# mcahny/vps

Measured on AMD Instinct MI355X. Metric: frames/sec FuseTrack 1024x2048, higher is better.
Workload: dtype f32-grade: f16x3 split operands (fp16 pair with scaled residual, 22 significand bits) on MFMA, f32 accumulate

## Files before the change

vps_amd/csrc/conv_common.h:

```cpp
#pragma once
#include "common.h"
#include "conv_plan.h"
#include <type_traits>
#include <cstdlib>

typedef float f32x16 __attribute__((ext_vector_type(16)));
typedef float f32x4 __attribute__((ext_vector_type(4)));

namespace {


constexpr int BM = 128;
constexpr int BK = 32;
constexpr int LDS_LD = 36;

template <bool X6, typename F>
void with_prec(const int prec, F&& f) {
    if (prec == VPS_PREC_BF16) f(std::integral_constant<int, VPS_PREC_BF16>{});
    else if (prec == VPS_PREC_BF16X3) f(std::integral_constant<int, VPS_PREC_BF16X3>{});
    else if (X6 && prec == VPS_PREC_BF16X6) f(std::integral_constant<int, X6 ? VPS_PREC_BF16X6 : VPS_PREC_F16X3>{});
    else f(std::integral_constant<int, VPS_PREC_F16X3>{});
}

struct RowInfo {
// ... 202 lines not shown
        for (int g = 0; g < 4; ++g)
#pragma unroll
            for (int e = 0; e < 4; ++e) {
                const int co = cbase + b * 32 + 8 * g + e;
                const bool cok = co < d.cout;
                const int cc = min(co, d.cout - 1);
                const float sc = d.scale ? d.scale[cc] : 1.f;
                const float sh = d.shift ? d.shift[cc] : 0.f;
                float rvs[TM];
#pragma unroll
                for (int a = 0; a < TM; ++a) rvs[a] = d_res ? d_res[rpix[a] * d.res_ld + d.res_coff + cc] : 0.f;
#pragma unroll
                for (int a = 0; a < TM; ++a) {
                    if (!inside[a] || !cok) continue;
                    const float t = acc[a][b][4 * g + e] * sc + sh + rvs[a];
                    d.out[opix[a] * d.out_ld + d.out_coff + co] = vps_act(t, d.act, d.slope);
                }
            }
}

typedef __bf16 bf16x8 __attribute__((ext_vector_type(8)));
typedef __bf16 bf16x4 __attribute__((ext_vector_type(4)));
template <class T> using vec8 = T __attribute__((ext_vector_type(8)));
template <class T> using vec4 = T __attribute__((ext_vector_type(4)));
typedef unsigned int u32x4 __attribute__((ext_vector_type(4)));

__device__ __forceinline__ __amdgpu_buffer_rsrc_t make_rsrc(const void* p, const unsigned bytes) {
    return __builtin_amdgcn_make_buffer_rsrc(const_cast<void*>(p), 0, (int)bytes, 0x00020000);
}
template <class V>
__device__ __forceinline__ V buffer_load16(const __amdgpu_buffer_rsrc_t r, const unsigned voff, const unsigned soff) {
    return __builtin_bit_cast(V, __builtin_amdgcn_raw_buffer_load_b128(r, (int)voff, (int)soff, 0));
}
constexpr int LDS_LDH = 32;
__device__ __forceinline__ int lds_swz(int row) { return (row >> 2) & 3; }

template <int MODE> struct Split;
template <> struct Split<VPS_PREC_BF16> {
    typedef __bf16 elem;
    static constexpr int NSA = 1, NSB = 1, NT = 1, NLB = 1;
    static constexpr int PA[6] = {0, 0, 0, 0, 0, 0};
    static constexpr int PB[6] = {0, 0, 0, 0, 0, 0};
};
template <> struct Split<VPS_PREC_BF16X3> {
    typedef __bf16 elem;
    static constexpr int NSA = 2, NSB = 2, NT = 3, NLB = 2;
    static constexpr int PA[6] = {1, 0, 0, 0, 0, 0};
    static constexpr int PB[6] = {0, 1, 0, 0, 0, 0};
};
template <> struct Split<VPS_PREC_BF16X6> {
    typedef __bf16 elem;
    static constexpr int NSA = 3, NSB = 3, NT = 6, NLB = 3;
    static constexpr int PA[6] = {2, 0, 1, 1, 0, 0};
    static constexpr int PB[6] = {0, 2, 1, 0, 1, 0};
};
template <> struct Split<VPS_PREC_F16X3> {
    typedef _Float16 elem;
    static constexpr int NSA = 2, NSB = 3, NT = 3, NLB = 2;
    static constexpr int PA[6] = {0, 1, 0, 0, 0, 0};
    static constexpr int PB[6] = {1, 2, 0, 0, 0, 0};
};

template <int MODE>
__device__ __forceinline__ vec8<typename Split<MODE>::elem> derive_weight_plane(const vec8<typename Split<MODE>::elem> g0) {
    static_assert(MODE == VPS_PREC_F16X3, "only the fp16 mode has a derived weight plane");
    typedef _Float16 h16x8 __attribute__((ext_vector_type(8)));
// ... 58 lines not shown
```

vps_amd/csrc/conv_h8.hip:

```cpp
#include "conv_common.h"

namespace {

template <int MODE, int KH, int KW>
__global__ __launch_bounds__(512, 2)
void conv_mfma_h8_kernel(const vps_conv_desc d, const int tiles_m, const int tiles_n, const int chunks_per_split) {
    constexpr int TM = 2, TN = 2, WAVES_N = 2, BN = 128;
    constexpr int NTAP = KH * KW;
    constexpr int HW = 32 + KW - 1, HH = 8 + KH - 1;
    constexpr int HROWS = HH * HW;
    constexpr int NLD = (HROWS + 63) / 64;
    typedef Split<MODE> SM;
    typedef typename SM::elem elem_t;
    typedef vec8<elem_t> x8;
    typedef vec4<elem_t> x4;
    constexpr int NSA = SM::NSA, NSB = SM::NSB;
    constexpr int PLANE = NLD * 64 * LDS_LDH;
    constexpr int ABUF = NSA * PLANE;
    constexpr int NLB = NSB;
    constexpr int NFRAG = NLB * 2 * (BN / 32);
    constexpr int BBUF = NFRAG * 512;
    static_assert((NFRAG * 64) % 512 == 0, "whole 16-byte chunks per thread");
    constexpr int NBL = NFRAG * 64 / 512;
    static_assert(2 * (ABUF + BBUF) * 2 <= 160 * 1024, "LDS budget of the CU");

    __shared__ __attribute__((aligned(16))) elem_t As[2 * ABUF];
    __shared__ __attribute__((aligned(16))) elem_t Bs[2 * BBUF];

    const int t = threadIdx.x;
    int swz = xcd_swizzle(blockIdx.x, gridDim.x);
    int tile_n, tile_m, cls, split;
    decode_tile(d, swz, tiles_n, tiles_m, tile_n, tile_m, cls, split);

    const int py = cls / d.os_x, px = cls - py * d.os_x;
    const int H = d.H, W = d.W, cin_pad = d.cin_pad;
    const int tiles_x = (d.Qw + 31) >> 5, tiles_y = (d.Qh + 7) >> 3;
    const int tx = tile_m % tiles_x, tq = tile_m / tiles_x;
    const int ty = tq % tiles_y, n = tq / tiles_y;
    const int iy_org = ty * 8 - d.pad_y[py], ix_org = tx * 32 - d.pad_x[px];
// ... 27 lines not shown
        const int iy = iy_org + hy, ix = ix_org + hx;
        const bool ok = hp < HROWS && (unsigned)iy < (unsigned)H && (unsigned)ix < (unsigned)W;
        hoff[i] = ok ? (unsigned)((n * H + iy) * W + ix) * ld4 + (unsigned)(d.in_coff + k4 * 4) * 4u : 0xFFFFFFF0u;
    }

    auto load_A = [&]() {
        const bool kv = achunk * BK + k4 * 4 < cin_pad;
        const unsigned coff = (unsigned)achunk * (BK * 4u);
        ++achunk;
#pragma unroll
        for (int i = 0; i < NLD; ++i)
            areg[i] = buffer_load16<f32x4>(arsrc, (kv && hoff[i] != 0xFFFFFFF0u) ? hoff[i] + coff : 0xFFFFFFF0u, 0u);
    };
    auto store_A = [&](int i, int buf) {
        x4 sp[NSA];
        split_act<MODE>(areg[i], sp, amax);
        const int row = r0 + 64 * i;
#pragma unroll
        for (int p = 0; p < NSA; ++p)
            *reinterpret_cast<x4*>(&As[buf * ABUF + p * PLANE + row * LDS_LDH + (((k4 >> 1) ^ lds_swz(row)) << 3) + ((k4 & 1) << 2)]) = sp[p];
    };
    auto load_B = [&](int step) {
#pragma unroll
        for (int j = 0; j < NBL; ++j) {
            const int f = __builtin_amdgcn_readfirstlane((t + 512 * j) >> 6), bcol = f % (BN / 32), pm = f / (BN / 32);
            breg[j] = buffer_load16<x8>(wrsrc, (unsigned)lane * 16u,
                                        wbase + (unsigned)(((size_t)(pm >> 1) * wplane + ((size_t)bcol * kst + 2 * step + (pm & 1)) * 512) * sizeof(elem_t)));
        }
    };
    auto store_B = [&](int buf) {
#pragma unroll
        for (int j = 0; j < NBL; ++j) *reinterpret_cast<x8*>(&Bs[buf * BBUF + (t + 512 * j) * 8]) = breg[j];
    };

    int hbase[TM];
#pragma unroll
    for (int a = 0; a < TM; ++a) hbase[a] = (wm * TM + a) * HW + (lane & 31);
    x8 af[2][NSA][TM];
    auto read_A = [&](int m, int buf, int toff) {
#pragma unroll
        for (int a = 0; a < TM; ++a) {
            const int hrow = hbase[a] + toff;
            const int off = buf * ABUF + hrow * LDS_LDH + (((2 * m + (lane >> 5)) ^ lds_swz(hrow)) << 3);
#pragma unroll
            for (int p = 0; p < NSA; ++p) af[m][p][a] = *reinterpret_cast<const x8*>(&As[off + p * PLANE]);
        }
    };
    x8 bcur[2][NSB][TN];
    auto read_B = [&](int m, int buf) {
#pragma unroll
        for (int p = 0; p < NLB; ++p)
#pragma unroll
            for (int b = 0; b < TN; ++b)
                bcur[m][p][b] = *reinterpret_cast<const x8*>(&Bs[buf * BBUF + (((p * 2 + m) * (BN / 32)) + wn * TN + b) * 512 + lane * 8]);
        if constexpr (NLB < NSB) {
#pragma unroll
            for (int b = 0; b < TN; ++b) bcur[m][2][b] = derive_weight_plane<MODE>(bcur[m][0][b]);
        }
    };

    f32x16 acc[TM][TN];
#pragma unroll
    for (int a = 0; a < TM; ++a)
#pragma unroll
        for (int b = 0; b < TN; ++b)
#pragma unroll
            for (int r = 0; r < 16; ++r) acc[a][b][r] = 0.f;

    load_A();
    load_B(0);
#pragma unroll
    for (int i = 0; i < NLD; ++i) store_A(i, 0);
    store_B(0);
    load_A();
    __syncthreads();

    constexpr int NT = SM::NT;
    constexpr int NMF = 2 * NT * TM * TN;
    constexpr int SPT = (NLD + NTAP - 2) / (NTAP - 1);
    constexpr int NW = SPT + 3;

    for (int chunk = 0; chunk < nchunks; ++chunk) {
        const int cur = chunk & 1;
#pragma unroll
        for (int tp = 0; tp < NTAP; ++tp) {
            const int step = chunk * NTAP + tp;
            const int bb = step & 1;
            const int bstep = min(step + 1, nsteps - 1);
            const int toff = (tp / KW) * HW + (tp % KW);
            read_A(0, cur, toff);
            read_B(0, bb);
            __builtin_amdgcn_sched_barrier(0);

            auto work = [&](const int w) {
                if (w == 0) load_B(bstep);
                else if (w == 1) { read_A(1, cur, toff); read_B(1, bb); }
                else if (w < SPT + 2) {
                    const int si = w - 2;
                    if (tp < NTAP - 1) {
                        const int row = tp * SPT + si;
                        if (row < NLD) store_A(row, cur ^ 1);
                    } else if (si == 0) load_A();
                } else store_B(bb ^ 1);
            };

            int mf = 0;
#pragma unroll
            for (int m = 0; m < 2; ++m)
#pragma unroll
                for (int q = 0; q < NT; ++q)
#pragma unroll
                    for (int a = 0; a < TM; ++a)
#pragma unroll
                        for (int b = 0; b < TN; ++b) {
                            acc[a][b] = split_mfma<MODE>(bcur[m][SM::PB[q]][b], af[m][SM::PA[q]][a], acc[a][b]);
                            ++mf;
#pragma unroll
                            for (int w = 0; w < NW; ++w) {
                                const int pos = ((w + 1) * NMF) / (NW + 1);
                                if (mf == (pos < 1 ? 1 : pos)) {
                                    __builtin_amdgcn_sched_barrier(0);
                                    work(w);
                                    __builtin_amdgcn_sched_barrier(0);
                                }
                            }
                        }
            __syncthreads();
        }
    }
    report_range<MODE>(d, amax);
    conv_epilogue<TM, TN, BN, true, 5>(d, acc, tiles_m * 256, tile_m, tile_n, cls, split, py, px, wm, wn, lane, (cls * tiles_m + tile_m) * tiles_n + tile_n);
}

struct S2Tap { int ph, j, i, idx, t, nt; };
constexpr int s2_taps_1d(int K, int a) { return (K - a + 1) / 2; }
constexpr S2Tap s2_tap(int K, int ts) {
    int base = 0;
    for (int ph = 0; ph < 4; ++ph) {
        const int a = ph >> 1, b = ph & 1, J = s2_taps_1d(K, a), I = s2_taps_1d(K, b);
        if (ts < base + J * I) {
            const int t = ts - base, j = t / I, i = t - j * I;
            return S2Tap{ph, j, i, (2 * j + a) * K + 2 * i + b, t, J * I};
        }
        base += J * I;
    }
    return S2Tap{0, 0, 0, 0, 0, 1};
}
template <int N, typename F>
__device__ __forceinline__ void static_for(F&& f) {
    if constexpr (N > 0) {
        static_for<N - 1>(f);
        f(std::integral_constant<int, N - 1>{});
    }
}

template <int MODE, int K, int BN = 128>
__global__ __launch_bounds__(512, 2)
void conv_mfma_h8s2_kernel(const vps_conv_desc d, const int tiles_m, const int tiles_n, const int chunks_per_split) {
    static_assert(BN == 128 || BN == 64, "two column waves of 64 or 32 columns");
    constexpr int TM = 2, TN = BN / 64, WAVES_N = 2;
    constexpr int NTAP = K * K;
    constexpr int J0 = s2_taps_1d(K, 0);
    constexpr int HW = 32 + J0 - 1, HH = 8 + J0 - 1;
    constexpr int HROWS = HH * HW;
    constexpr int NLD = (HROWS + 63) / 64;
    typedef Split<MODE> SM;
    typedef typename SM::elem elem_t;
    typedef vec8<elem_t> x8;
    typedef vec4<elem_t> x4;
    constexpr int NSA = SM::NSA, NSB = SM::NSB;
    constexpr int PLANE = NLD * 64 * LDS_LDH;
    constexpr int ABUF = NSA * PLANE;
    constexpr int NLB = NSB;
    constexpr int NFRAG = NLB * 2 * (BN / 32);
    constexpr int NBL = (NFRAG * 64 + 511) / 512;
    constexpr bool WHOLE = (NFRAG * 64) % 512 == 0;
    constexpr int BBUF = NBL * 512 * 8;
    static_assert(2 * (ABUF + BBUF) * 2 <= 160 * 1024, "LDS budget of the CU");

    __shared__ __attribute__((aligned(16))) elem_t As[2 * ABUF];
    __shared__ __attribute__((aligned(16))) elem_t Bs[2 * BBUF];

    const int t = threadIdx.x;
    const int swz = xcd_swizzle(blockIdx.x, gridDim.x);
    int tile_n, tile_m, cls, split;
    decode_tile(d, swz, tiles_n, tiles_m, tile_n, tile_m, cls, split);

    const int H = d.H, W = d.W, cin_pad = d.cin_pad;
    const int tiles_x = (d.Qw + 31) >> 5, tiles_y = (d.Qh + 7) >> 3;
    const int tx = tile_m % tiles_x, tq = tile_m / tiles_x;
    const int ty = tq % tiles_y, n = tq / tiles_y;
// ... 27 lines not shown
        const unsigned coff = (unsigned)(d.in_coff + cic) * 4u;
        if (++aph == 4) { aph = 0; ++achunk; }
#pragma unroll
        for (int i = 0; i < NLD; ++i) {
            const int hp = r0 + 64 * i;
            const int hy = hp / HW, hx = hp - hy * HW;
            const int iy = iy_org + a + 2 * hy, ix = ix_org + b + 2 * hx;
            const bool ok = kv && hy < rows && hx < cols && (unsigned)iy < (unsigned)H && (unsigned)ix < (unsigned)W;
            areg[i] = buffer_load16<f32x4>(arsrc, ok ? (unsigned)((n * H + iy) * W + ix) * ld4 + coff : 0xFFFFFFF0u, 0u);
        }
    };
    auto store_A = [&](int i, int buf) {
        x4 sp[NSA];
        split_act<MODE>(areg[i], sp, amax);
        const int row = r0 + 64 * i;
#pragma unroll
        for (int p = 0; p < NSA; ++p)
            *reinterpret_cast<x4*>(&As[buf * ABUF + p * PLANE + row * LDS_LDH + (((k4 >> 1) ^ lds_swz(row)) << 3) + ((k4 & 1) << 2)]) = sp[p];
    };
    auto load_B = [&](int wstep) {
#pragma unroll
        for (int j = 0; j < NBL; ++j) {
            const int fr = __builtin_amdgcn_readfirstlane((t + 512 * j) >> 6), f = WHOLE ? fr : min(fr, NFRAG - 1);
            const int bcol = f % (BN / 32), pm = f / (BN / 32);
            breg[j] = buffer_load16<x8>(wrsrc, (unsigned)lane * 16u,
                                        wbase + (unsigned)(((size_t)(pm >> 1) * wplane + ((size_t)bcol * kst + 2 * wstep + (pm & 1)) * 512) * sizeof(elem_t)));
        }
    };
    auto store_B = [&](int buf) {
#pragma unroll
        for (int j = 0; j < NBL; ++j)
            *reinterpret_cast<x8*>(&Bs[buf * BBUF + (t + 512 * j) * 8]) = breg[j];
    };

    int hbase[TM];
#pragma unroll
    for (int a = 0; a < TM; ++a) hbase[a] = (wm * TM + a) * HW + (lane & 31);
    x8 af[2][NSA][TM];
    auto read_A = [&](int m, int buf, int toff) {
#pragma unroll
        for (int a = 0; a < TM; ++a) {
            const int hrow = hbase[a] + toff;
            const int off = buf * ABUF + hrow * LDS_LDH + (((2 * m + (lane >> 5)) ^ lds_swz(hrow)) << 3);
#pragma unroll
            for (int p = 0; p < NSA; ++p) af[m][p][a] = *reinterpret_cast<const x8*>(&As[off + p * PLANE]);
        }
    };
    x8 bcur[2][NSB][TN];
    auto read_B = [&](int m, int buf) {
#pragma unroll
        for (int p = 0; p < NLB; ++p)
#pragma unroll
            for (int b = 0; b < TN; ++b)
                bcur[m][p][b] = *reinterpret_cast<const x8*>(&Bs[buf * BBUF + (((p * 2 + m) * (BN / 32)) + wn * TN + b) * 512 + lane * 8]);
        if constexpr (NLB < NSB) {
#pragma unroll
            for (int b = 0; b < TN; ++b) bcur[m][2][b] = derive_weight_plane<MODE>(bcur[m][0][b]);
        }
    };

    f32x16 acc[TM][TN];
#pragma unroll
    for (int a = 0; a < TM; ++a)
#pragma unroll
        for (int b = 0; b < TN; ++b)
#pragma unroll
            for (int r = 0; r < 16; ++r) acc[a][b][r] = 0.f;

    load_A();
    load_B(s2_tap(K, 0).idx);
#pragma unroll
    for (int i = 0; i < NLD; ++i) store_A(i, 0);
    store_B(0);
    load_A();
    __syncthreads();

    constexpr int NT = SM::NT;
    constexpr int NMF = 2 * NT * TM * TN;

    for (int chunk = 0; chunk < nchunks; ++chunk) {
        static_for<NTAP>([&](auto ts_tag) {
            constexpr int TS = decltype(ts_tag)::value;
            constexpr S2Tap tp = s2_tap(K, TS);
            constexpr S2Tap nx = s2_tap(K, (TS + 1) % NTAP);
            constexpr int cur = tp.ph & 1;
            constexpr bool last_of_phase = tp.t == tp.nt - 1;
            constexpr int SPT = (NLD + tp.nt - 1) / tp.nt;
            constexpr int NW = 3 + SPT + (last_of_phase ? 1 : 0);
            const int step = chunk * NTAP + TS;
            const int bb = step & 1;
            const int wnext = (TS + 1 < NTAP ? chunk : min(chunk + 1, nchunks - 1)) * NTAP + nx.idx;
            constexpr int toff = tp.j * HW + tp.i;
            read_A(0, cur, toff);
            read_B(0, bb);
            __builtin_amdgcn_sched_barrier(0);

            auto work = [&](const int w) {
                if (w == 0) load_B(wnext);
                else if (w == 1) { read_A(1, cur, toff); read_B(1, bb); }
                else if (w < SPT + 2) {
                    const int row = tp.t * SPT + (w - 2);
                    if (row < NLD) store_A(row, cur ^ 1);
                } else if (last_of_phase && w == SPT + 2) load_A();
                else store_B(bb ^ 1);
            };

            int mf = 0;
#pragma unroll
            for (int m = 0; m < 2; ++m)
#pragma unroll
                for (int q = 0; q < NT; ++q)
#pragma unroll
                    for (int a = 0; a < TM; ++a)
#pragma unroll
                        for (int b = 0; b < TN; ++b) {
                            acc[a][b] = split_mfma<MODE>(bcur[m][SM::PB[q]][b], af[m][SM::PA[q]][a], acc[a][b]);
                            ++mf;
#pragma unroll
                            for (int w = 0; w < NW; ++w) {
                                const int pos = ((w + 1) * NMF) / (NW + 1);
                                if (mf == (pos < 1 ? 1 : pos)) {
                                    __builtin_amdgcn_sched_barrier(0);
                                    work(w);
                                    __builtin_amdgcn_sched_barrier(0);
                                }
                            }
                        }
            __syncthreads();
        });
    }
    report_range<MODE>(d, amax);
    conv_epilogue<TM, TN, BN, true, 5>(d, acc, tiles_m * 256, tile_m, tile_n, cls, split, 0, 0, wm, wn, lane, (cls * tiles_m + tile_m) * tiles_n + tile_n);
}

}

__attribute__((visibility("hidden")))
void vpsi_launch_conv_h8(const vps_conv_desc& d, const conv_plan& p, hipStream_t s) {
    with_prec<false>(d.prec, [&](auto mode) {
        constexpr int MODE = decltype(mode)::value;
        if (d.KH == 3) hipLaunchKernelGGL((conv_mfma_h8_kernel<MODE, 3, 3>), dim3(p.grid), dim3(p.block), 0, s, d, p.tiles_m, p.tiles_n, p.chunks_per_split);
        else hipLaunchKernelGGL((conv_mfma_h8_kernel<MODE, 2, 2>), dim3(p.grid), dim3(p.block), 0, s, d, p.tiles_m, p.tiles_n, p.chunks_per_split);
    });
}

__attribute__((visibility("hidden")))
void vpsi_launch_conv_h8s2(const vps_conv_desc& d, const conv_plan& p, hipStream_t s) {
    with_prec<false>(d.prec, [&](auto mode) {
        constexpr int MODE = decltype(mode)::value;
#define VPS_H8S2_LAUNCH(K, BN) \
    hipLaunchKernelGGL((conv_mfma_h8s2_kernel<MODE, K, BN>), dim3(p.grid), dim3(p.block), 0, s, d, p.tiles_m, p.tiles_n, p.chunks_per_split)
        if (d.KH == 3) { if (d.tile_n == 64) VPS_H8S2_LAUNCH(3, 64); else VPS_H8S2_LAUNCH(3, 128); }
        else { if (d.tile_n == 64) VPS_H8S2_LAUNCH(5, 64); else VPS_H8S2_LAUNCH(5, 128); }
#undef VPS_H8S2_LAUNCH
    });
}
```

vps_amd/csrc/conv_h8p.hip:

```cpp
#include "conv_common.h"

namespace {

template <int N, typename F>
__device__ __forceinline__ void static_for_p(F&& f) {
    if constexpr (N > 0) {
        static_for_p<N - 1>(f);
        f(std::integral_constant<int, N - 1>{});
    }
}

template <int MODE, int KH, int KW>
__global__ __launch_bounds__(512, 2)
void conv_mfma_h8p_kernel(const vps_conv_desc d, const int tiles_m, const int tiles_n, const int chunks_per_split) {
    constexpr int TM = 2, TN = 2, WAVES_N = 2, BN = 128;
    constexpr int NTAP = KH * KW;
    static_assert(NTAP % 3 == 0 || NTAP == 4, "ring / register-set index of a tap must be static: 9 taps (9 % 3 == 0) or 4 taps (12-step cycle handled by the caller)");
    constexpr int HW = 32 + KW - 1, HH = 8 + KH - 1;
    constexpr int HROWS = HH * HW;
    constexpr int NLD = (HROWS + 63) / 64;
    typedef Split<MODE> SM;
    typedef typename SM::elem elem_t;
    typedef vec8<elem_t> x8;
    typedef vec4<elem_t> x4;
    constexpr int NSA = SM::NSA, NSB = SM::NSB, NLB = SM::NLB, NT = SM::NT;
    constexpr int PLANE = HROWS * LDS_LDH;
    constexpr int ABUF = NSA * PLANE;
    constexpr int NFRAG = NSB * 2 * (BN / 32);
    constexpr int BBUF = NFRAG * 512;
    static_assert(NFRAG * 64 == NSB * 512, "thread t stages chunk t of every plane");
    static_assert((2 * ABUF + 3 * BBUF) * 2 <= 160 * 1024, "LDS budget of the CU");

    __shared__ __attribute__((aligned(16))) elem_t As[2 * ABUF];
    __shared__ __attribute__((aligned(16))) elem_t Bs[3 * BBUF];

    const int t = threadIdx.x;
    int swz = xcd_swizzle(blockIdx.x, gridDim.x);
    int tile_n, tile_m, cls, split;
    decode_tile(d, swz, tiles_n, tiles_m, tile_n, tile_m, cls, split);

    const int py = cls / d.os_x, px = cls - py * d.os_x;
    const int H = d.H, W = d.W, cin_pad = d.cin_pad;
    const int tiles_x = (d.Qw + 31) >> 5, tiles_y = (d.Qh + 7) >> 3;
    const int tx = tile_m % tiles_x, tq = tile_m / tiles_x;
    const int ty = tq % tiles_y, n = tq / tiles_y;
    const int iy_org = ty * 8 - d.pad_y[py], ix_org = tx * 32 - d.pad_x[px];

    const int k4 = t & 7;
    const int r0 = t >> 3;
    const int chunk0 = split * chunks_per_split;
    const int nchunks = min(chunks_per_split, d.kpad / (BK * NTAP) - chunk0);
    const int nsteps = nchunks * NTAP;

    const int lane = t & 63;
    const int wave = __builtin_amdgcn_readfirstlane(t >> 6);
    const int wm = wave / WAVES_N, wn = wave - wm * WAVES_N;
    const int nbt = d.cout_pad >> 5, kst = d.kpad >> 4;
    const size_t wplane = (size_t)d.nclass * nbt * kst * 512;
    const __amdgpu_buffer_rsrc_t wrsrc = make_rsrc(d.w_split, (unsigned)(wplane * NSB * sizeof(elem_t)));
    const unsigned wbase = (unsigned)((((size_t)(cls * nbt + tile_n * (BN / 32)) * kst + 2 * (size_t)chunk0 * NTAP) * 512) * sizeof(elem_t));
    const __amdgpu_buffer_rsrc_t arsrc = make_rsrc(d.in, (unsigned)((size_t)d.N * H * W * d.in_ld * sizeof(float)));
    const unsigned ld4 = (unsigned)d.in_ld * 4u;

    f32x4 areg[NLD];
    int achunk = chunk0;
    x8 breg[3][NLB];
    float amax = 0.f;

    unsigned hoff[NLD];
#pragma unroll
    for (int i = 0; i < NLD; ++i) {
        const int hp = r0 + 64 * i;
        const int hy = hp / HW, hx = hp - hy * HW;
        const int iy = iy_org + hy, ix = ix_org + hx;
        const bool ok = hp < HROWS && (unsigned)iy < (unsigned)H && (unsigned)ix < (unsigned)W;
        hoff[i] = ok ? (unsigned)((n * H + iy) * W + ix) * ld4 + (unsigned)(d.in_coff + k4 * 4) * 4u : 0xFFFFFFF0u;
    }

    auto load_A = [&]() {
        const bool kv = achunk * BK + k4 * 4 < cin_pad;
        const unsigned coff = (unsigned)achunk * (BK * 4u);
        ++achunk;
#pragma unroll
        for (int i = 0; i < NLD; ++i)
            areg[i] = buffer_load16<f32x4>(arsrc, (kv && hoff[i] != 0xFFFFFFF0u) ? hoff[i] + coff : 0xFFFFFFF0u, 0u);
    };
    auto store_A = [&](const int i, const int buf) {
        x4 sp[NSA];
        split_act<MODE>(areg[i], sp, amax);
        const int row = r0 + 64 * i;
        if (row < HROWS) {
#pragma unroll
            for (int p = 0; p < NSA; ++p)
                *reinterpret_cast<x4*>(&As[buf * ABUF + p * PLANE + row * LDS_LDH + (((k4 >> 1) ^ lds_swz(row)) << 3) + ((k4 & 1) << 2)]) = sp[p];
        }
    };
    auto load_B = [&](const int step, const int set) {
        const int sc = min(step, nsteps - 1);
        const int f = wave, bcol = f % (BN / 32), slab = f / (BN / 32);
#pragma unroll
        for (int p = 0; p < NLB; ++p)
            breg[set][p] = buffer_load16<x8>(wrsrc, (unsigned)lane * 16u,
                                             wbase + (unsigned)(((size_t)p * wplane + ((size_t)bcol * kst + 2 * sc + slab) * 512) * sizeof(elem_t)));
    };
    auto store_B = [&](const int slot, const int set) {
#pragma unroll
        for (int p = 0; p < NLB; ++p) *reinterpret_cast<x8*>(&Bs[slot * BBUF + (t + 512 * p) * 8]) = breg[set][p];
        if constexpr (NLB < NSB) *reinterpret_cast<x8*>(&Bs[slot * BBUF + (t + 512 * NLB) * 8]) = derive_weight_plane<MODE>(breg[set][0]);
    };

    int hbase[TM];
#pragma unroll
    for (int a = 0; a < TM; ++a) hbase[a] = (wm * TM + a) * HW + (lane & 31);
    x8 af[2][NSA][TM];
    x8 bcur[2][NSB][TN];
    constexpr int NRD = NSA * TM + NSB * TN;
    auto read_frag = [&](const int j, const int m, const int abuf, const int toff, const int slot) {
        if (j < NSA * TM) {
            const int p = j / TM, a = j - p * TM;
            const int hrow = hbase[a] + toff;
            af[m][p][a] = *reinterpret_cast<const x8*>(&As[abuf * ABUF + p * PLANE + hrow * LDS_LDH + (((2 * m + (lane >> 5)) ^ lds_swz(hrow)) << 3)]);
        } else {
            const int jj = j - NSA * TM, p = jj / TN, b = jj - p * TN;
            bcur[m][p][b] = *reinterpret_cast<const x8*>(&Bs[slot * BBUF + (((p * 2 + m) * (BN / 32)) + wn * TN + b) * 512 + lane * 8]);
        }
    };

    f32x16 acc[TM][TN];
#pragma unroll
    for (int a = 0; a < TM; ++a)
#pragma unroll
        for (int b = 0; b < TN; ++b)
#pragma unroll
            for (int r = 0; r < 16; ++r) acc[a][b][r] = 0.f;

    load_A();
    load_B(0, 0);
    load_B(1, 1);
#pragma unroll
    for (int i = 0; i < NLD; ++i) store_A(i, 0);
    store_B(0, 0);
    store_B(1, 1);
    load_B(2, 2);
    load_A();
    __syncthreads();
#pragma unroll
    for (int j = 0; j < NRD; ++j) read_frag(j, 0, 0, 0, 0);

    constexpr int NMS = NT * TM * TN;
    constexpr int STG = NTAP / 2;
    constexpr int SPT = (NLD + STG - 1) / STG;
    auto mfma = [&](const int m, const int i) {
        const int q = i / (TM * TN), r = i - q * (TM * TN), a = r / TN, b = r - a * TN;
        acc[a][b] = split_mfma<MODE>(bcur[m][SM::PB[q]][b], af[m][SM::PA[q]][a], acc[a][b]);
    };

    auto tap = [&](const int chunk, auto tp_tag, auto r3_tag) {
        constexpr int tp = decltype(tp_tag)::value;
        constexpr int R3 = decltype(r3_tag)::value;
        const int cur = chunk & 1;
        const int step = chunk * NTAP + tp;
        constexpr int toff = (tp / KW) * HW + (tp % KW);
        constexpr int ntp = (tp + 1) % NTAP;
        constexpr int ntoff = (ntp / KW) * HW + (ntp % KW);
        const int nbuf = tp == NTAP - 1 ? cur ^ 1 : cur;
#pragma unroll
        for (int i = 0; i < NMS; ++i) {
            mfma(0, i);
            __builtin_amdgcn_sched_barrier(0);
            if (i == 0) load_B(step + 3, R3);
#pragma unroll
            for (int j = 0; j < NRD; ++j)
                if ((j * (NMS - 1)) / NRD + 1 == i || (NMS == 1 && i == 0)) read_frag(j, 1, cur, toff, R3);
            __builtin_amdgcn_sched_barrier(0);
        }
#pragma unroll
        for (int i = 0; i < NMS; ++i) {
            mfma(1, i);
            __builtin_amdgcn_sched_barrier(0);
            if (tp < STG) {
#pragma unroll
                for (int si = 0; si < SPT; ++si)
                    if (i == (si * NMS) / (SPT + 1) && tp * SPT + si < NLD) store_A(tp * SPT + si, cur ^ 1);
            }
            if (i == (SPT * NMS) / (SPT + 1)) {
                store_B((R3 + 2) % 3, (R3 + 2) % 3);
                if (tp == STG) load_A();
            }
#pragma unroll
            for (int j = 0; j < NRD; ++j)
                if ((j * (NMS - 1)) / NRD + 1 == i || (NMS == 1 && i == 0)) read_frag(j, 0, nbuf, ntoff, (R3 + 1) % 3);
            __builtin_amdgcn_sched_barrier(0);
        }
        __syncthreads();
    };

    if constexpr (NTAP % 3 == 0) {
        for (int chunk = 0; chunk < nchunks; ++chunk)
            static_for_p<NTAP>([&](auto tpc) {
                constexpr int TP = decltype(tpc)::value;
                tap(chunk, std::integral_constant<int, TP>{}, std::integral_constant<int, TP % 3>{});
            });
    } else {
        int chunk = 0;
        for (; chunk + 2 < nchunks; chunk += 3)
            static_for_p<3 * NTAP>([&](auto sc) {
                constexpr int S = decltype(sc)::value;
                tap(chunk + S / NTAP, std::integral_constant<int, S % NTAP>{}, std::integral_constant<int, S % 3>{});
            });
        if (chunk < nchunks) {
            static_for_p<NTAP>([&](auto sc) {
                constexpr int S = decltype(sc)::value;
                tap(chunk, std::integral_constant<int, S>{}, std::integral_constant<int, S % 3>{});
            });
            ++chunk;
            if (chunk < nchunks)
                static_for_p<NTAP>([&](auto sc) {
                    constexpr int S = decltype(sc)::value;
                    tap(chunk, std::integral_constant<int, S>{}, std::integral_constant<int, (NTAP + S) % 3>{});
                });
        }
    }
    report_range<MODE>(d, amax);
    conv_epilogue<TM, TN, BN, true, 5>(d, acc, tiles_m * 256, tile_m, tile_n, cls, split, py, px, wm, wn, lane, (cls * tiles_m + tile_m) * tiles_n + tile_n);
}

}

__attribute__((visibility("hidden")))
void vpsi_launch_conv_h8p(const vps_conv_desc& d, const conv_plan& p, hipStream_t s) {
    hipLaunchKernelGGL((conv_mfma_h8p_kernel<VPS_PREC_F16X3, 3, 3>), dim3(p.grid), dim3(p.block), 0, s, d, p.tiles_m, p.tiles_n, p.chunks_per_split);
}
```

vps_amd/csrc/conv_mfma.hip:

```cpp
#include "conv_common.h"

namespace {
template <int TM, int TN, int WAVES_M, int WAVES_N, bool DEFORM>
__global__ __launch_bounds__(256, 2)
void conv_mfma_f32_kernel(const vps_conv_desc d, const int M, const int tiles_m, const int tiles_n,
                          const int ksteps_per_split) {
    constexpr int BN = WAVES_N * TN * 32;
    static_assert(WAVES_M * TM * 32 == BM, "block M tile must be 128");
    static_assert(WAVES_M * WAVES_N == 4, "4 wavefronts per block");
    constexpr int NB = BN / 32;

    __shared__ __attribute__((aligned(16))) float As[BM * LDS_LD];
    __shared__ __attribute__((aligned(16))) float Bs[BN * LDS_LD];

    const int t = threadIdx.x;
    int swz = xcd_swizzle(blockIdx.x, gridDim.x);
    int tile_n, tile_m, cls, split;
    decode_tile(d, swz, tiles_n, tiles_m, tile_n, tile_m, cls, split);

    const int py = cls / d.os_x, px = cls - py * d.os_x;
    const int pad_y = d.pad_y[py], pad_x = d.pad_x[px];
    const float* __restrict__ wcls = d.w + (size_t)cls * d.cout_pad * d.kpad;

    const int H = d.H, W = d.W, KH = d.KH, KW = d.KW, cin_pad = d.cin_pad;
// ... 701 lines not shown
}

template <int TM, int TN, int WAVES_M, int WAVES_N>
void launch_conv(const vps_conv_desc& d, const conv_plan& p, hipStream_t s) {
    const dim3 grid(p.grid), block(p.block);
    if (p.kernel == CONV_K_HALO) {
        with_prec<true>(d.prec, [&](auto mode) {
            constexpr int MODE = decltype(mode)::value;
            if (d.KH == 3) hipLaunchKernelGGL((conv_mfma_bf16h_kernel<TM, TN, WAVES_M, WAVES_N, MODE, 3, 3>), grid, block, 0, s, d, p.tiles_m, p.tiles_n, p.chunks_per_split);
            else hipLaunchKernelGGL((conv_mfma_bf16h_kernel<TM, TN, WAVES_M, WAVES_N, MODE, 2, 2>), grid, block, 0, s, d, p.tiles_m, p.tiles_n, p.chunks_per_split);
        });
        return;
    }
#define VPS_CONV_LAUNCH(KERNEL) hipLaunchKernelGGL((KERNEL), grid, block, 0, s, d, p.M, p.tiles_m, p.tiles_n, p.per_split)
    if (p.kernel == CONV_K_F32) {
        if (d.offset) VPS_CONV_LAUNCH((conv_mfma_f32_kernel<TM, TN, WAVES_M, WAVES_N, true>));
        else VPS_CONV_LAUNCH((conv_mfma_f32_kernel<TM, TN, WAVES_M, WAVES_N, false>));
        return;
    }
    const bool tapmajor = d.korder == 0 && d.KH * d.KW > 1;
    with_prec<true>(d.prec, [&](auto mode) {
        constexpr int MODE = decltype(mode)::value;
        if (d.offset) VPS_CONV_LAUNCH((conv_mfma_bf16p_kernel<TM, TN, WAVES_M, WAVES_N, MODE, false, true>));
        else if (tapmajor) VPS_CONV_LAUNCH((conv_mfma_bf16p_kernel<TM, TN, WAVES_M, WAVES_N, MODE, true>));
        else VPS_CONV_LAUNCH((conv_mfma_bf16p_kernel<TM, TN, WAVES_M, WAVES_N, MODE, false>));
    });
#undef VPS_CONV_LAUNCH
}

conv_switches conv_switches_now(const vps_conv_desc& d) {
    const auto on = [](const char* name) { const char* const e = getenv(name); return !(e && atoi(e) == 0); };
    const auto not0 = [](const char* name) { const char* const e = getenv(name); return !(e && e[0] == '0'); };
    static const bool s2_halo = not0("VPS_S2_HALO"), thin = on("VPS_THIN"), debug_occ = getenv("VPS_DEBUG_OCC") != nullptr;
    conv_switches sw = {true, true, true, true, s2_halo, thin, debug_occ};
    if (d.prec != VPS_PREC_F16X3) return sw;
    if (d.tile_n == 32) {
        if (d.cout > 16) sw.n32 = not0("VPS_N32");
        else if (d.nclass == 4) sw.n16t = on("VPS_N16T");
    } else if (d.tile_n <= 128 && d.KH == 1) sw.pw = on("VPS_PW");
    else if (d.tile_n == 128 && d.KH == 3 && d.stride == 1) sw.h8p = on("VPS_H8P");
    return sw;
}

const conv_limits& conv_limits_once(const bool debug) {
    static const conv_limits lim = [debug] {
        conv_limits l = {};
        int dev = 0;
        (void)hipGetDevice(&dev);
        (void)hipDeviceGetAttribute(&l.cus, hipDeviceAttributeMultiprocessorCount, dev);
        vpsi_conv_pw_limits(l, debug);
        vpsi_conv_thin_limits(l, debug);
        if (debug) vpsi_conv_q_debug_occ();
        return l;
    }();
    return lim;
}

}

extern "C" int vps_conv2d(const vps_conv_desc* dp, void* stream) {
    if (!dp) return VPS_EARG(1);
    const vps_conv_desc& d = *dp;
    if (const int e = vpsi_conv_check(d)) return e;
    const conv_switches sw = conv_switches_now(d);
    const conv_plan p = vpsi_conv_plan(d, conv_limits_once(sw.debug_occ), sw);
    hipStream_t s = (hipStream_t)stream;
    switch (p.kernel) {
        case CONV_K_NONE: return p.err;
        case CONV_K_SMALL3X3V: case CONV_K_SMALL_BATCHED: case CONV_K_SMALL: vpsi_launch_conv_small(d, p, s); break;
        case CONV_K_THIN: vpsi_launch_conv_thin(d, p, s); break;
        case CONV_K_DCN256:
            hipLaunchKernelGGL((conv_mfma_bf16p_kernel<2, 4, 2, 2, VPS_PREC_F16X3, false, true>), dim3(p.grid), dim3(p.block), 0, s, d, p.M, p.tiles_m, p.tiles_n, p.per_split);
            break;
        case CONV_K_N16T: case CONV_K_N32: case CONV_K_N16: vpsi_launch_conv_n16(d, p, s); break;
        case CONV_K_H8S2: vpsi_launch_conv_h8s2(d, p, s); break;
        case CONV_K_H8P: vpsi_launch_conv_h8p(d, p, s); break;
        case CONV_K_H8: vpsi_launch_conv_h8(d, p, s); break;
        case CONV_K_PW: vpsi_launch_conv_pw(d, p, s); break;
        case CONV_K_Q: vpsi_launch_conv_q(d, p, s); break;
        default:
            if (d.tile_n == 128) launch_conv<2, 2, 2, 2>(d, p, s);
            else if (d.tile_n == 64) launch_conv<2, 1, 2, 2>(d, p, s);
            else launch_conv<1, 1, 4, 1>(d, p, s);
    }
    int st = vps_launch_status();
    if (st || !p.needs_reduce) return st;
    const size_t total = (size_t)d.nclass * p.M * d.cout;
    if (p.reduce_v4) hipLaunchKernelGGL(conv_splitk_reduce_kernel<4>, dim3(stream_grid((long)(total / 4), 256)), dim3(256), 0, s, d, p.M);
    else hipLaunchKernelGGL(conv_splitk_reduce_kernel<1>, dim3(stream_grid((long)total, 256)), dim3(256), 0, s, d, p.M);
    return vps_launch_status();
}
```

vps_amd/csrc/conv_plan.h:

```cpp
#pragma once
#include <stddef.h>
#include "../../include/vps_hip.h"

#ifndef VPS_EARG
#define VPS_EARG(x) (-1000 - (x))
#endif

enum conv_kernel {
    CONV_K_NONE = 0,
    CONV_K_SMALL3X3V,
    CONV_K_SMALL_BATCHED,
    CONV_K_SMALL,
    CONV_K_THIN,
    CONV_K_DCN256,
    CONV_K_N16T,
    CONV_K_N32,
    CONV_K_N16,
    CONV_K_H8S2,
    CONV_K_H8P,
    CONV_K_H8,
    CONV_K_HALO,
    CONV_K_PW,
    CONV_K_Q,
    CONV_K_F32,
// ... 2 lines not shown

struct conv_plan {
    int kernel;
    int err;
    int M;
    int tiles_m, tiles_n;
    int per_split;
    int chunks_per_split;
    unsigned grid, block;
    size_t smem;
    int nk, nit;
    int G, logG, nslot;
    int runs_per_row, total_runs;
    int thin;
    int ntiles;
    bool needs_reduce;
    bool reduce_v4;
};

struct conv_limits {
    int cus;
    int pw_per_cu[2];
    int thin_per_cu[4];
};

struct conv_switches {
    bool pw;
    bool h8p;
    bool n16t;
    bool n32;
    bool s2_halo;
    bool thin;
    bool debug_occ;
};

struct conv_thin_shape { int c4, ks, s, ph; };
extern const conv_thin_shape conv_thin_shapes[4];

int vpsi_conv_check(const vps_conv_desc& d);
conv_plan vpsi_conv_plan(const vps_conv_desc& d, const conv_limits& lim, const conv_switches& sw);
const char* vpsi_conv_kernel_name(int kernel);

#ifdef __HIPCC__
void vpsi_launch_conv_small(const vps_conv_desc& d, const conv_plan& p, hipStream_t s);
void vpsi_launch_conv_thin(const vps_conv_desc& d, const conv_plan& p, hipStream_t s);
void vpsi_launch_conv_n16(const vps_conv_desc& d, const conv_plan& p, hipStream_t s);
void vpsi_launch_conv_h8(const vps_conv_desc& d, const conv_plan& p, hipStream_t s);
void vpsi_launch_conv_h8p(const vps_conv_desc& d, const conv_plan& p, hipStream_t s);
void vpsi_launch_conv_h8s2(const vps_conv_desc& d, const conv_plan& p, hipStream_t s);
void vpsi_launch_conv_pw(const vps_conv_desc& d, const conv_plan& p, hipStream_t s);
void vpsi_launch_conv_q(const vps_conv_desc& d, const conv_plan& p, hipStream_t s);
void vpsi_conv_pw_limits(conv_limits& lim, bool debug);
void vpsi_conv_thin_limits(conv_limits& lim, bool debug);
void vpsi_conv_q_debug_occ();
#endif
```

Measured before the change: 56.42.

## Stream conv weight tiles straight from global memory into LDS in h8 kernels

```diff
diff --git a/vps_amd/csrc/conv_common.h b/vps_amd/csrc/conv_common.h
--- a/vps_amd/csrc/conv_common.h
+++ b/vps_amd/csrc/conv_common.h
@@ -258,6 +258,21 @@
 __device__ __forceinline__ V buffer_load16(const __amdgpu_buffer_rsrc_t r, const unsigned voff, const unsigned soff) {
     return __builtin_bit_cast(V, __builtin_amdgcn_raw_buffer_load_b128(r, (int)voff, (int)soff, 0));
 }
+__device__ __forceinline__ void glds16(const void* const gbase, const unsigned voff, const unsigned lds_dst) {
+    unsigned keep;
+    asm volatile("s_mov_b32 %0, m0\n\ts_mov_b32 m0, %3\n\ts_nop 0\n\tglobal_load_lds_dwordx4 %1, %2\n\ts_mov_b32 m0, %0"
+                 : "=&s"(keep) : "v"(voff), "s"(gbase), "s"(lds_dst) : "memory");
+}
+template <class T>
+__device__ __forceinline__ unsigned lds_addr(const T* const p) {
+    return (unsigned)__builtin_amdgcn_readfirstlane((int)(size_t)(const __attribute__((address_space(3))) T*)p);
+}
+template <int N>
+__device__ __forceinline__ void wait_vm() {
+    static_assert(N >= 0 && N < 64, "6-bit counter");
+    __builtin_amdgcn_s_waitcnt(0x0F70 | (N & 15) | ((N >> 4) << 14));
+}
+
 constexpr int LDS_LDH = 32;
 __device__ __forceinline__ int lds_swz(int row) { return (row >> 2) & 3; }
 
diff --git a/vps_amd/csrc/conv_h8.hip b/vps_amd/csrc/conv_h8.hip
--- a/vps_amd/csrc/conv_h8.hip
+++ b/vps_amd/csrc/conv_h8.hip
@@ -2,9 +2,8 @@
 
 namespace {
 
-template <int MODE, int KH, int KW>
-__global__ __launch_bounds__(512, 2)
-void conv_mfma_h8_kernel(const vps_conv_desc d, const int tiles_m, const int tiles_n, const int chunks_per_split) {
+template <int MODE, int KH, int KW, bool WDMA>
+__device__ __forceinline__ void conv_h8_body(const vps_conv_desc& d, const int tiles_m, const int tiles_n, const int chunks_per_split) {
     constexpr int TM = 2, TN = 2, WAVES_N = 2, BN = 128;
     constexpr int NTAP = KH * KW;
     constexpr int HW = 32 + KW - 1, HH = 8 + KH - 1;
@@ -98,6 +97,15 @@
 #pragma unroll
         for (int j = 0; j < NBL; ++j) *reinterpret_cast<x8*>(&Bs[buf * BBUF + (t + 512 * j) * 8]) = breg[j];
     };
+    const char* const wsrc = reinterpret_cast<const char*>(d.w_split) + wbase;
+    auto dma_B = [&](int step, int buf) {
+#pragma unroll
+        for (int j = 0; j < NBL; ++j) {
+            const int f = wave + 8 * j, bcol = f % (BN / 32), pm = f / (BN / 32);
+            glds16(wsrc + ((size_t)(pm >> 1) * wplane + ((size_t)bcol * kst + 2 * step + (pm & 1)) * 512) * sizeof(elem_t), (unsigned)lane * 16u,
+                   lds_addr(&Bs[buf * BBUF + f * 512]));
+        }
+    };
 
     int hbase[TM];
 #pragma unroll
@@ -134,11 +142,13 @@
             for (int r = 0; r < 16; ++r) acc[a][b][r] = 0.f;
 
     load_A();
-    load_B(0);
+    if constexpr (WDMA) dma_B(0, 0);
+    else load_B(0);
 #pragma unroll
     for (int i = 0; i < NLD; ++i) store_A(i, 0);
-    store_B(0);
+    if constexpr (!WDMA) store_B(0);
     load_A();
+    if constexpr (WDMA) wait_vm<NLD>();
     __syncthreads();
 
     constexpr int NT = SM::NT;
@@ -159,7 +169,10 @@
             __builtin_amdgcn_sched_barrier(0);
 
             auto work = [&](const int w) {
-                if (w == 0) load_B(bstep);
+                if (w == 0) {
+                    if constexpr (WDMA) dma_B(bstep, bb ^ 1);
+                    else load_B(bstep);
+                }
                 else if (w == 1) { read_A(1, cur, toff); read_B(1, bb); }
                 else if (w < SPT + 2) {
                     const int si = w - 2;
@@ -167,7 +180,7 @@
                         const int row = tp * SPT + si;
                         if (row < NLD) store_A(row, cur ^ 1);
                     } else if (si == 0) load_A();
-                } else store_B(bb ^ 1);
+                } else if constexpr (!WDMA) store_B(bb ^ 1);
             };
 
             int mf = 0;
@@ -191,11 +204,26 @@
                                 }
                             }
                         }
+            if constexpr (WDMA) {
+                if (tp == NTAP - 1) wait_vm<NLD>();
+                else wait_vm<0>();
+            }
             __syncthreads();
         }
     }
     report_range<MODE>(d, amax);
     conv_epilogue<TM, TN, BN, true, 5>(d, acc, tiles_m * 256, tile_m, tile_n, cls, split, py, px, wm, wn, lane, (cls * tiles_m + tile_m) * tiles_n + tile_n);
+}
+
+template <int MODE, int KH, int KW>
+__global__ __launch_bounds__(512, 2)
+void conv_mfma_h8_kernel(const vps_conv_desc d, const int tiles_m, const int tiles_n, const int chunks_per_split) {
+    conv_h8_body<MODE, KH, KW, true>(d, tiles_m, tiles_n, chunks_per_split);
+}
+template <int MODE, int KH, int KW>
+__global__ __launch_bounds__(512, 2)
+void conv_mfma_h8_wreg_kernel(const vps_conv_desc d, const int tiles_m, const int tiles_n, const int chunks_per_split) {
+    conv_h8_body<MODE, KH, KW, false>(d, tiles_m, tiles_n, chunks_per_split);
 }
 
 struct S2Tap { int ph, j, i, idx, t, nt; };
@@ -220,9 +248,8 @@
     }
 }
 
-template <int MODE, int K, int BN = 128>
-__global__ __launch_bounds__(512, 2)
-void conv_mfma_h8s2_kernel(const vps_conv_desc d, const int tiles_m, const int tiles_n, const int chunks_per_split) {
+template <int MODE, int K, int BN, bool WDMA>
+__device__ __forceinline__ void conv_h8s2_body(const vps_conv_desc& d, const int tiles_m, const int tiles_n, const int chunks_per_split) {
     static_assert(BN == 128 || BN == 64, "two column waves of 64 or 32 columns");
     constexpr int TM = 2, TN = BN / 64, WAVES_N = 2;
     constexpr int NTAP = K * K;
@@ -316,6 +343,16 @@
         for (int j = 0; j < NBL; ++j)
             *reinterpret_cast<x8*>(&Bs[buf * BBUF + (t + 512 * j) * 8]) = breg[j];
     };
+    const char* const wsrc = reinterpret_cast<const char*>(d.w_split) + wbase;
+    auto dma_B = [&](int wstep, int buf) {
+#pragma unroll
+        for (int j = 0; j < NBL; ++j) {
+            const int fr = wave + 8 * j, f = WHOLE ? fr : min(fr, NFRAG - 1);
+            const int bcol = f % (BN / 32), pm = f / (BN / 32);
+            glds16(wsrc + ((size_t)(pm >> 1) * wplane + ((size_t)bcol * kst + 2 * wstep + (pm & 1)) * 512) * sizeof(elem_t), (unsigned)lane * 16u,
+                   lds_addr(&Bs[buf * BBUF + fr * 512]));
+        }
+    };
 
     int hbase[TM];
 #pragma unroll
@@ -352,11 +389,13 @@
             for (int r = 0; r < 16; ++r) acc[a][b][r] = 0.f;
 
     load_A();
-    load_B(s2_tap(K, 0).idx);
+    if constexpr (WDMA) dma_B(s2_tap(K, 0).idx, 0);
+    else load_B(s2_tap(K, 0).idx);
 #pragma unroll
     for (int i = 0; i < NLD; ++i) store_A(i, 0);
-    store_B(0);
+    if constexpr (!WDMA) store_B(0);
     load_A();
+    if constexpr (WDMA) wait_vm<NLD>();
     __syncthreads();
 
     constexpr int NT = SM::NT;
@@ -380,13 +419,16 @@
             __builtin_amdgcn_sched_barrier(0);
 
             auto work = [&](const int w) {
-                if (w == 0) load_B(wnext);
+                if (w == 0) {
+                    if constexpr (WDMA) dma_B(wnext, bb ^ 1);
+                    else load_B(wnext);
+                }
                 else if (w == 1) { read_A(1, cur, toff); read_B(1, bb); }
                 else if (w < SPT + 2) {
                     const int row = tp.t * SPT + (w - 2);
                     if (row < NLD) store_A(row, cur ^ 1);
                 } else if (last_of_phase && w == SPT + 2) load_A();
-                else store_B(bb ^ 1);
+                else if constexpr (!WDMA) store_B(bb ^ 1);
             };
 
             int mf = 0;
@@ -410,6 +452,7 @@
                                 }
                             }
                         }
+            if constexpr (WDMA) wait_vm<last_of_phase ? NLD : 0>();
             __syncthreads();
         });
     }
@@ -417,23 +460,40 @@
     conv_epilogue<TM, TN, BN, true, 5>(d, acc, tiles_m * 256, tile_m, tile_n, cls, split, 0, 0, wm, wn, lane, (cls * tiles_m + tile_m) * tiles_n + tile_n);
 }
 
+template <int MODE, int K, int BN = 128>
+__global__ __launch_bounds__(512, 2)
+void conv_mfma_h8s2_kernel(const vps_conv_desc d, const int tiles_m, const int tiles_n, const int chunks_per_split) {
+    conv_h8s2_body<MODE, K, BN, K == 5>(d, tiles_m, tiles_n, chunks_per_split);
+}
+template <int MODE, int K, int BN = 128>
+__global__ __launch_bounds__(512, 2)
+void conv_mfma_h8s2_wreg_kernel(const vps_conv_desc d, const int tiles_m, const int tiles_n, const int chunks_per_split) {
+    conv_h8s2_body<MODE, K, BN, false>(d, tiles_m, tiles_n, chunks_per_split);
+}
+
 }
 
 __attribute__((visibility("hidden")))
-void vpsi_launch_conv_h8(const vps_conv_desc& d, const conv_plan& p, hipStream_t s) {
+void vpsi_launch_conv_h8(const vps_conv_desc& d, const conv_plan& p, const bool w_regs, hipStream_t s) {
     with_prec<false>(d.prec, [&](auto mode) {
         constexpr int MODE = decltype(mode)::value;
-        if (d.KH == 3) hipLaunchKernelGGL((conv_mfma_h8_kernel<MODE, 3, 3>), dim3(p.grid), dim3(p.block), 0, s, d, p.tiles_m, p.tiles_n, p.chunks_per_split);
-        else hipLaunchKernelGGL((conv_mfma_h8_kernel<MODE, 2, 2>), dim3(p.grid), dim3(p.block), 0, s, d, p.tiles_m, p.tiles_n, p.chunks_per_split);
+#define VPS_H8_LAUNCH(K, KERNEL) \
+    hipLaunchKernelGGL((KERNEL<MODE, K, K>), dim3(p.grid), dim3(p.block), 0, s, d, p.tiles_m, p.tiles_n, p.chunks_per_split)
+        if (d.KH == 3) { if (w_regs) VPS_H8_LAUNCH(3, conv_mfma_h8_wreg_kernel); else VPS_H8_LAUNCH(3, conv_mfma_h8_kernel); }
+        else { if (w_regs) VPS_H8_LAUNCH(2, conv_mfma_h8_wreg_kernel); else VPS_H8_LAUNCH(2, conv_mfma_h8_kernel); }
+#undef VPS_H8_LAUNCH
     });
 }
 
 __attribute__((visibility("hidden")))
-void vpsi_launch_conv_h8s2(const vps_conv_desc& d, const conv_plan& p, hipStream_t s) {
+void vpsi_launch_conv_h8s2(const vps_conv_desc& d, const conv_plan& p, const bool w_regs, hipStream_t s) {
     with_prec<false>(d.prec, [&](auto mode) {
         constexpr int MODE = decltype(mode)::value;
 #define VPS_H8S2_LAUNCH(K, BN) \
-    hipLaunchKernelGGL((conv_mfma_h8s2_kernel<MODE, K, BN>), dim3(p.grid), dim3(p.block), 0, s, d, p.tiles_m, p.tiles_n, p.chunks_per_split)
+    do { \
+        if (w_regs && K == 5) hipLaunchKernelGGL((conv_mfma_h8s2_wreg_kernel<MODE, 5, BN>), dim3(p.grid), dim3(p.block), 0, s, d, p.tiles_m, p.tiles_n, p.chunks_per_split); \
+        else hipLaunchKernelGGL((conv_mfma_h8s2_kernel<MODE, K, BN>), dim3(p.grid), dim3(p.block), 0, s, d, p.tiles_m, p.tiles_n, p.chunks_per_split); \
+    } while (0)
         if (d.KH == 3) { if (d.tile_n == 64) VPS_H8S2_LAUNCH(3, 64); else VPS_H8S2_LAUNCH(3, 128); }
         else { if (d.tile_n == 64) VPS_H8S2_LAUNCH(5, 64); else VPS_H8S2_LAUNCH(5, 128); }
 #undef VPS_H8S2_LAUNCH
diff --git a/vps_amd/csrc/conv_h8p.hip b/vps_amd/csrc/conv_h8p.hip
--- a/vps_amd/csrc/conv_h8p.hip
+++ b/vps_amd/csrc/conv_h8p.hip
@@ -10,9 +10,8 @@
     }
 }
 
-template <int MODE, int KH, int KW>
-__global__ __launch_bounds__(512, 2)
-void conv_mfma_h8p_kernel(const vps_conv_desc d, const int tiles_m, const int tiles_n, const int chunks_per_split) {
+template <int MODE, int KH, int KW, bool WDMA>
+__device__ __forceinline__ void conv_h8p_body(const vps_conv_desc& d, const int tiles_m, const int tiles_n, const int chunks_per_split) {
     constexpr int TM = 2, TN = 2, WAVES_N = 2, BN = 128;
     constexpr int NTAP = KH * KW;
     static_assert(NTAP % 3 == 0 || NTAP == 4, "ring / register-set index of a tap must be static: 9 taps (9 % 3 == 0) or 4 taps (12-step cycle handled by the caller)");
@@ -64,7 +63,7 @@
 
     f32x4 areg[NLD];
     int achunk = chunk0;
-    x8 breg[3][NLB];
+    x8 breg[WDMA ? 1 : 3][NLB];
     float amax = 0.f;
 
     unsigned hoff[NLD];
@@ -107,6 +106,16 @@
 #pragma unroll
         for (int p = 0; p < NLB; ++p) *reinterpret_cast<x8*>(&Bs[slot * BBUF + (t + 512 * p) * 8]) = breg[set][p];
         if constexpr (NLB < NSB) *reinterpret_cast<x8*>(&Bs[slot * BBUF + (t + 512 * NLB) * 8]) = derive_weight_plane<MODE>(breg[set][0]);
+    };
+
+    const char* const wsrc = reinterpret_cast<const char*>(d.w_split) + wbase;
+    auto dma_B = [&](const int step, const int slot) {
+        const int sc = min(step, nsteps - 1);
+        const int f = wave, bcol = f % (BN / 32), slab = f / (BN / 32);
+#pragma unroll
+        for (int p = 0; p < NSB; ++p)
+            glds16(wsrc + ((size_t)p * wplane + ((size_t)bcol * kst + 2 * sc + slab) * 512) * sizeof(elem_t), (unsigned)lane * 16u,
+                   lds_addr(&Bs[slot * BBUF + (wave * 64 + 512 * p) * 8]));
     };
 
     int hbase[TM];
@@ -135,14 +144,17 @@
             for (int r = 0; r < 16; ++r) acc[a][b][r] = 0.f;
 
     load_A();
-    load_B(0, 0);
-    load_B(1, 1);
+    if constexpr (WDMA) { dma_B(0, 0); dma_B(1, 1); }
+    else { load_B(0, 0); load_B(1, 1); }
 #pragma unroll
     for (int i = 0; i < NLD; ++i) store_A(i, 0);
-    store_B(0, 0);
-    store_B(1, 1);
-    load_B(2, 2);
+    if constexpr (!WDMA) {
+        store_B(0, 0);
+        store_B(1, 1);
+        load_B(2, 2);
+    }
     load_A();
+    if constexpr (WDMA) wait_vm<NLD>();
     __syncthreads();
 #pragma unroll
     for (int j = 0; j < NRD; ++j) read_frag(j, 0, 0, 0, 0);
@@ -168,7 +180,10 @@
         for (int i = 0; i < NMS; ++i) {
             mfma(0, i);
             __builtin_amdgcn_sched_barrier(0);
-            if (i == 0) load_B(step + 3, R3);
+            if (i == 0) {
+                if constexpr (WDMA) dma_B(step + 2, (R3 + 2) % 3);
+                else load_B(step + 3, R3);
+            }
 #pragma unroll
             for (int j = 0; j < NRD; ++j)
                 if ((j * (NMS - 1)) / NRD + 1 == i || (NMS == 1 && i == 0)) read_frag(j, 1, cur, toff, R3);
@@ -184,7 +199,7 @@
                     if (i == (si * NMS) / (SPT + 1) && tp * SPT + si < NLD) store_A(tp * SPT + si, cur ^ 1);
             }
             if (i == (SPT * NMS) / (SPT + 1)) {
-                store_B((R3 + 2) % 3, (R3 + 2) % 3);
+                if constexpr (!WDMA) store_B((R3 + 2) % 3, (R3 + 2) % 3);
                 if (tp == STG) load_A();
             }
 #pragma unroll
@@ -192,6 +207,7 @@
                 if ((j * (NMS - 1)) / NRD + 1 == i || (NMS == 1 && i == 0)) read_frag(j, 0, nbuf, ntoff, (R3 + 1) % 3);
             __builtin_amdgcn_sched_barrier(0);
         }
+        if constexpr (WDMA) wait_vm<tp == STG ? NLD : 0>();
         __syncthreads();
     };
 
@@ -225,9 +241,21 @@
     conv_epilogue<TM, TN, BN, true, 5>(d, acc, tiles_m * 256, tile_m, tile_n, cls, split, py, px, wm, wn, lane, (cls * tiles_m + tile_m) * tiles_n + tile_n);
 }
 
+template <int MODE, int KH, int KW>
+__global__ __launch_bounds__(512, 2)
+void conv_mfma_h8p_kernel(const vps_conv_desc d, const int tiles_m, const int tiles_n, const int chunks_per_split) {
+    conv_h8p_body<MODE, KH, KW, true>(d, tiles_m, tiles_n, chunks_per_split);
+}
+template <int MODE, int KH, int KW>
+__global__ __launch_bounds__(512, 2)
+void conv_mfma_h8p_wreg_kernel(const vps_conv_desc d, const int tiles_m, const int tiles_n, const int chunks_per_split) {
+    conv_h8p_body<MODE, KH, KW, false>(d, tiles_m, tiles_n, chunks_per_split);
+}
+
 }
 
 __attribute__((visibility("hidden")))
-void vpsi_launch_conv_h8p(const vps_conv_desc& d, const conv_plan& p, hipStream_t s) {
-    hipLaunchKernelGGL((conv_mfma_h8p_kernel<VPS_PREC_F16X3, 3, 3>), dim3(p.grid), dim3(p.block), 0, s, d, p.tiles_m, p.tiles_n, p.chunks_per_split);
-}
+void vpsi_launch_conv_h8p(const vps_conv_desc& d, const conv_plan& p, const bool w_regs, hipStream_t s) {
+    if (w_regs) hipLaunchKernelGGL((conv_mfma_h8p_wreg_kernel<VPS_PREC_F16X3, 3, 3>), dim3(p.grid), dim3(p.block), 0, s, d, p.tiles_m, p.tiles_n, p.chunks_per_split);
+    else hipLaunchKernelGGL((conv_mfma_h8p_kernel<VPS_PREC_F16X3, 3, 3>), dim3(p.grid), dim3(p.block), 0, s, d, p.tiles_m, p.tiles_n, p.chunks_per_split);
+}
diff --git a/vps_amd/csrc/conv_mfma.hip b/vps_amd/csrc/conv_mfma.hip
--- a/vps_amd/csrc/conv_mfma.hip
+++ b/vps_amd/csrc/conv_mfma.hip
@@ -757,7 +757,8 @@
     const auto on = [](const char* name) { const char* const e = getenv(name); return !(e && atoi(e) == 0); };
     const auto not0 = [](const char* name) { const char* const e = getenv(name); return !(e && e[0] == '0'); };
     static const bool s2_halo = not0("VPS_S2_HALO"), thin = on("VPS_THIN"), debug_occ = getenv("VPS_DEBUG_OCC") != nullptr;
-    conv_switches sw = {true, true, true, true, s2_halo, thin, debug_occ};
+    conv_switches sw = {true, true, true, true, s2_halo, thin, debug_occ, false};
+    if (d.tile_n >= 64 && d.KH > 1 && d.prec != VPS_PREC_F32) sw.w_regs = !on("VPS_WDMA");
     if (d.prec != VPS_PREC_F16X3) return sw;
     if (d.tile_n == 32) {
         if (d.cout > 16) sw.n32 = not0("VPS_N32");
@@ -798,9 +799,9 @@
             hipLaunchKernelGGL((conv_mfma_bf16p_kernel<2, 4, 2, 2, VPS_PREC_F16X3, false, true>), dim3(p.grid), dim3(p.block), 0, s, d, p.M, p.tiles_m, p.tiles_n, p.per_split);
             break;
         case CONV_K_N16T: case CONV_K_N32: case CONV_K_N16: vpsi_launch_conv_n16(d, p, s); break;
-        case CONV_K_H8S2: vpsi_launch_conv_h8s2(d, p, s); break;
-        case CONV_K_H8P: vpsi_launch_conv_h8p(d, p, s); break;
-        case CONV_K_H8: vpsi_launch_conv_h8(d, p, s); break;
+        case CONV_K_H8S2: vpsi_launch_conv_h8s2(d, p, sw.w_regs, s); break;
+        case CONV_K_H8P: vpsi_launch_conv_h8p(d, p, sw.w_regs, s); break;
+        case CONV_K_H8: vpsi_launch_conv_h8(d, p, sw.w_regs, s); break;
         case CONV_K_PW: vpsi_launch_conv_pw(d, p, s); break;
         case CONV_K_Q: vpsi_launch_conv_q(d, p, s); break;
         default:
diff --git a/vps_amd/csrc/conv_plan.h b/vps_amd/csrc/conv_plan.h
--- a/vps_amd/csrc/conv_plan.h
+++ b/vps_amd/csrc/conv_plan.h
@@ -58,6 +58,7 @@
     bool s2_halo;
     bool thin;
     bool debug_occ;
+    bool w_regs;
 };
 
 struct conv_thin_shape { int c4, ks, s, ph; };
@@ -71,9 +72,9 @@
 void vpsi_launch_conv_small(const vps_conv_desc& d, const conv_plan& p, hipStream_t s);
 void vpsi_launch_conv_thin(const vps_conv_desc& d, const conv_plan& p, hipStream_t s);
 void vpsi_launch_conv_n16(const vps_conv_desc& d, const conv_plan& p, hipStream_t s);
-void vpsi_launch_conv_h8(const vps_conv_desc& d, const conv_plan& p, hipStream_t s);
-void vpsi_launch_conv_h8p(const vps_conv_desc& d, const conv_plan& p, hipStream_t s);
-void vpsi_launch_conv_h8s2(const vps_conv_desc& d, const conv_plan& p, hipStream_t s);
+void vpsi_launch_conv_h8(const vps_conv_desc& d, const conv_plan& p, bool w_regs, hipStream_t s);
+void vpsi_launch_conv_h8p(const vps_conv_desc& d, const conv_plan& p, bool w_regs, hipStream_t s);
+void vpsi_launch_conv_h8s2(const vps_conv_desc& d, const conv_plan& p, bool w_regs, hipStream_t s);
 void vpsi_launch_conv_pw(const vps_conv_desc& d, const conv_plan& p, hipStream_t s);
 void vpsi_launch_conv_q(const vps_conv_desc& d, const conv_plan& p, hipStream_t s);
 void vpsi_conv_pw_limits(conv_limits& lim, bool debug);
```

Result: no change. 56.60, median of 6 (+0.3%).
